# YufengJin/BundleSDF

Measured on AMD Instinct MI355X. Metric: NeRF training rays/sec + ms/iter, 64-frame pool, 2048 rays/frame, higher is better.
Workload: dtype fp16 table+MLP (MFMA) / fp32 accumulate+Adam (amp)

## Files before the change

bundlesdf_amd/csrc/field_step.hip:

```cpp
#include <algorithm>
#include <cstdlib>
#include <cstring>
#include <array>
#include <type_traits>
#include <vector>

#include "nof_device.h"
#include "ray_trace.h"
#include "mlp_lds.h"

#pragma clang fp contract(off)

#ifndef NOF_ABLATE
#define NOF_ABLATE 0
#endif
#define ABL(bits) (NOF_ABLATE && (a.ablate & (bits)))
#define ABL_HOST(d, bits) (NOF_ABLATE && ((d)->ablate & (bits)))
#define ABL_SKIPQ(q) ((q) < 2 ? (1 << (23 + (q))) : (1 << (27 + (q))))

namespace nof {

typedef _Float16 h8v __attribute__((ext_vector_type(8)));
typedef float f16v __attribute__((ext_vector_type(16)));

// ... 279 lines not shown
            const bool hit = !done && rem <= len;
            res = hit ? zin + rem : res;
            rem = done || hit ? rem : rem - len;
            done = done || hit;
            prev_out = zout;
        }
        if (!__any(!done)) return res;
    }
    for (; i < Kmax; ++i) {
        const float zin = __uint_as_float(bq[2 * i]), zout = __uint_as_float(bq[2 * i + 1]);
        if (zin == 0.f) return done ? res : ((rem <= eps && i >= 1) ? prev_out : 0.f);
        const float len = zout - zin;
        const bool hit = !done && rem <= len;
        res = hit ? zin + rem : res;
        rem = done || hit ? rem : rem - len;
        done = done || hit;
        prev_out = zout;
    }
    return done ? res : (rem <= eps ? __uint_as_float(bq[(Kmax - 1) * 2 + 1]) : 0.f);
}

__device__ __forceinline__ float bell_weight(const FieldArgs &a, float depth, float z) {
    if (depth > a.far_sc) return 0.f;
    const float u = (depth - z) / a.trunc;
    float w = sigmoidf(u * a.lambda) * sigmoidf(-u * a.lambda);
    const float dz = z - depth;
    const bool m = (dz <= a.trunc * a.ntr) && (dz >= -a.trunc);
    return m ? w : 0.f;
}

struct LevelInfo { float scale; uint32_t res, off, hs; };
__device__ __forceinline__ LevelInfo level_info(const FieldArgs &a, int lv) {
    const float4 v = a.levels[lv];
    return {v.x, __float_as_uint(v.y), __float_as_uint(v.z), __float_as_uint(v.w)};
}
__device__ __forceinline__ LevelInfo level_info_uniform(const FieldArgs &a, int lv) {
    const ConstU32 p = (ConstU32)(size_t)(a.levels + lv);
    return {__uint_as_float(p[0]), p[1], p[2], p[3]};
}

__device__ __forceinline__ __amdgpu_buffer_rsrc_t table_rsrc(const void *table) {
    return __builtin_amdgcn_make_buffer_rsrc(const_cast<void *>(table), (short)0, 0x7fffffff, 0x00020000);
}
typedef uint32_t u2v __attribute__((ext_vector_type(2)));
typedef uint32_t u4v __attribute__((ext_vector_type(4)));
__device__ __forceinline__ uint2 table_pair16(__amdgpu_buffer_rsrc_t rsrc, uint32_t row) {
    const u2v v = __builtin_amdgcn_raw_buffer_load_b64(rsrc, row * 4u, 0, 0);
    return make_uint2(v.x, v.y);
}

__device__ __forceinline__ uint32_t mul24(uint32_t a, uint32_t b) {
    uint32_t d;
    asm("v_mul_u32_u24 %0, %1, %2" : "=v"(d) : "v"(a), "v"(b));
    return d;
}
__device__ __forceinline__ uint32_t mad24(uint32_t a, uint32_t b, uint32_t c) {
    uint32_t d;
    asm("v_mad_u32_u24 %0, %1, %2, %3" : "=v"(d) : "v"(a), "v"(b), "v"(c));
    return d;
}
__device__ __forceinline__ bool level_dense_v(uint32_t rs, uint32_t hs) {
    return rs <= 1625u && mul24(mul24(rs, rs), rs) <= hs;
}
__device__ __forceinline__ uint32_t dense_base_v(uint32_t off, const uint32_t pg[3], uint32_t rs) {
    return off + pg[0] + mul24(mad24(pg[2], rs, pg[1]), rs);
}
__device__ __forceinline__ bool level_dense(uint32_t rs, uint32_t hs) { return (uint64_t)rs * rs * rs <= hs; }

__device__ __forceinline__ void corner_rows(const LevelInfo &li, const uint32_t pg[3], uint32_t rows[8]) {
    const uint32_t rs = li.res + 1;
    if (level_dense(rs, li.hs)) {
        const uint32_t base = dense_base_v(li.off, pg, rs), rs2 = rs * rs;
#pragma unroll
        for (int idx = 0; idx < 8; ++idx)
            rows[idx] = base + (idx & 1) + ((idx >> 1) & 1 ? rs : 0u) + ((idx >> 2) & 1 ? rs2 : 0u);
    } else {
#pragma unroll
        for (int idx = 0; idx < 8; ++idx) {
            uint32_t pl[3];
#pragma unroll
            for (int d = 0; d < 3; ++d) pl[d] = pg[d] + ((idx >> d) & 1);
            rows[idx] = li.off + grid_row<3>(0, false, li.hs, li.res, pl);
        }
    }
}

template <typename TT, bool PAIRED = false>
__device__ __forceinline__ void gather_level(const FieldArgs &a, const LevelInfo &li, const float x01[3], float pos[3],
                                             float e[8][2], uint32_t rows[8]) {
    const TT *tab = reinterpret_cast<const TT *>(a.table);
    uint32_t pg[3];
#pragma unroll
    for (int d = 0; d < 3; ++d) {
        pos[d] = __builtin_fmaf(x01[d], li.scale, 0.5f);
        pg[d] = (uint32_t)floorf(pos[d]);
        pos[d] -= (float)pg[d];
    }
    corner_rows(li, pg, rows);
    const uint32_t rs = li.res + 1;
    if (PAIRED && level_dense(rs, li.hs)) {
#pragma unroll
        for (int idx = 0; idx < 8; idx += 2) {
            const TT *p = tab + (size_t)rows[idx] * 2;
            if constexpr (sizeof(TT) == 4) {
                typedef float f4a __attribute__((ext_vector_type(4), aligned(8)));
                const f4a v = *reinterpret_cast<const f4a *>(p);
                e[idx][0] = v.x; e[idx][1] = v.y; e[idx + 1][0] = v.z; e[idx + 1][1] = v.w;
            } else {
                uint2 v;
                __builtin_memcpy(&v, p, 8);
                const __half2 h0 = __builtin_bit_cast(__half2, v.x), h1 = __builtin_bit_cast(__half2, v.y);
                e[idx][0] = __low2float(h0); e[idx][1] = __high2float(h0);
                e[idx + 1][0] = __low2float(h1); e[idx + 1][1] = __high2float(h1);
            }
        }
    } else {
#pragma unroll
        for (int idx = 0; idx < 8; ++idx) {
            const TT *p = tab + (size_t)rows[idx] * 2;
            if constexpr (sizeof(TT) == 4) {
                const float2 v = *reinterpret_cast<const float2 *>(p);
                e[idx][0] = v.x; e[idx][1] = v.y;
            } else {
                const __half2 v = *reinterpret_cast<const __half2 *>(p);
                e[idx][0] = __low2float(v); e[idx][1] = __high2float(v);
            }
        }
    }
}

template <typename TT>
__device__ __forceinline__ void encode_level(const FieldArgs &a, const LevelInfo &li, const float x01[3], float f[2]) {
    float pos[3], e[8][2];
    uint32_t rows[8];
    gather_level<TT, true>(a, li, x01, pos, e, rows);
    f[0] = 0.f; f[1] = 0.f;
#pragma unroll
    for (int idx = 0; idx < 8; ++idx) {
        float w = 1.f;
#pragma unroll
        for (int d = 0; d < 3; ++d) w *= ((idx >> d) & 1) ? pos[d] : 1 - pos[d];
        f[0] = __builtin_fmaf(w, e[idx][0], f[0]);
        f[1] = __builtin_fmaf(w, e[idx][1], f[1]);
    }
}

template <int CTRL> __device__ __forceinline__ int dpp_i(int v) {
    return __builtin_amdgcn_update_dpp(0, v, CTRL, 0xf, 0xf, true);
}
#define DPP_ROW_SHL(n) (0x100 + (n))
#define DPP_ROW_SHR(n) (0x110 + (n))

constexpr uint32_t SLOT_EMPTY = 0xffffffffu;

__device__ __forceinline__ uint32_t lds_cas(uint32_t *p, uint32_t key) {
    uint32_t e = SLOT_EMPTY;
    __hip_atomic_compare_exchange_strong(p, &e, key, __ATOMIC_RELAXED, __ATOMIC_RELAXED, __HIP_MEMORY_SCOPE_WORKGROUP);
    return e;
}

template <bool F16V> __device__ __forceinline__ uint32_t *slot_key(uint32_t *keys, uint32_t s) {
    return keys + (F16V ? 2 * s : s);
}
__device__ __forceinline__ void lds_add_h2(void *vals, uint32_t s, uint32_t packed) {
    __builtin_amdgcn_ds_atomic_fadd_v2f16(
        (__attribute__((address_space(3))) h2v *)(reinterpret_cast<uint32_t *>(vals) + 2 * s),
        __builtin_bit_cast(h2v, packed));
}
template <bool F16V>
__device__ __forceinline__ void lds_add(void *vals, uint32_t s, float v0, float v1) {
    if constexpr (F16V) {
        lds_add_h2(vals, s, __builtin_bit_cast(uint32_t, h2v{(_Float16)v0, (_Float16)v1}));
    } else {
        float *f = reinterpret_cast<float *>(vals) + 2 * s;
        __hip_atomic_fetch_add(f, v0, __ATOMIC_RELAXED, __HIP_MEMORY_SCOPE_WORKGROUP);
        __hip_atomic_fetch_add(f + 1, v1, __ATOMIC_RELAXED, __HIP_MEMORY_SCOPE_WORKGROUP);
    }
}

template <bool F16V>
__device__ __forceinline__ bool lds_probe(uint32_t *keys, void *vals, uint32_t mask, uint32_t key, float v0, float v1,
                                          float *g32, __half *g16) {
    uint32_t s = key;
#pragma unroll 1
    for (int p = 1; p < 16; ++p) {
        s = (s + 1) & mask;
        const uint32_t old = lds_cas(slot_key<F16V>(keys, s), key);
        if (old == SLOT_EMPTY || old == key) {
            lds_add<F16V>(vals, s, v0, v1);
            return true;
        }
    }
    if (g16) atomic_add_h2(g16 + (size_t)key * 2, v0, v1);
    else { atomic_add_f32(g32 + (size_t)key * 2, v0); atomic_add_f32(g32 + (size_t)key * 2 + 1, v1); }
    return false;
}

__device__ __forceinline__ void gather_level_t16(const FieldArgs &a, const LevelInfo &li, h2v g01, float t[8],
                                                 const uint32_t rows[8]) {
    const __half *tab = reinterpret_cast<const __half *>(a.table);
    const uint32_t rs = li.res + 1;
    if (level_dense(rs, li.hs)) {
#pragma unroll
        for (int idx = 0; idx < 8; idx += 2) {
            uint2 v;
            __builtin_memcpy(&v, tab + (size_t)rows[idx] * 2, 8);
            t[idx] = __builtin_amdgcn_fdot2(__builtin_bit_cast(h2v, v.x), g01, 0.f, false);
            t[idx + 1] = __builtin_amdgcn_fdot2(__builtin_bit_cast(h2v, v.y), g01, 0.f, false);
        }
    } else {
#pragma unroll
        for (int idx = 0; idx < 8; ++idx) {
            const uint32_t v = *reinterpret_cast<const uint32_t *>(tab + (size_t)rows[idx] * 2);
            t[idx] = __builtin_amdgcn_fdot2(__builtin_bit_cast(h2v, v), g01, 0.f, false);
        }
    }
}

template <typename TT, bool F16V>
__device__ __forceinline__ void backward_level(const FieldArgs &a, const LevelInfo &li, bool member, bool active,
                                               uint32_t part, const float x01[3], float g0, float g1, h2v g01,
                                               float gx[3], int lane, uint32_t *keys, void *vals, uint32_t mask,
                                               float *g32, __half *g16, int &n_direct) {
    float pos[3];
    uint32_t pg[3], crow[8];
#pragma unroll
    for (int d = 0; d < 3; ++d) {
        pos[d] = __builtin_fmaf(x01[d], li.scale, 0.5f);
        pg[d] = (uint32_t)pos[d];
        pos[d] = __builtin_amdgcn_fractf(pos[d]);
    }
    corner_rows(li, pg, crow);
    if (active && !a.no_dx) {
        float t[8];
        if constexpr (sizeof(TT) == 2) {
            gather_level_t16(a, li, g01, t, crow);
        } else {
            float e[8][2], pos_unused[3];
            uint32_t rows_unused[8];
            gather_level<TT, true>(a, li, x01, pos_unused, e, rows_unused);
#pragma unroll
            for (int k = 0; k < 8; ++k) t[k] = __builtin_fmaf(g1, e[k][1], g0 * e[k][0]);
        }
        float dx[4], ax[4];
#pragma unroll
        for (int j = 0; j < 4; ++j) {
            dx[j] = t[2 * j + 1] - t[2 * j];
            ax[j] = __builtin_fmaf(pos[0], dx[j], t[2 * j]);
        }
        float dy[2], by[2], ux[2];
#pragma unroll
        for (int z = 0; z < 2; ++z) {
            dy[z] = ax[2 * z + 1] - ax[2 * z];
            by[z] = __builtin_fmaf(pos[1], dy[z], ax[2 * z]);
            ux[z] = __builtin_fmaf(pos[1], dx[2 * z + 1] - dx[2 * z], dx[2 * z]);
        }
        gx[0] = __builtin_fmaf(li.scale, __builtin_fmaf(pos[2], ux[1] - ux[0], ux[0]), gx[0]);
        gx[1] = __builtin_fmaf(li.scale, __builtin_fmaf(pos[2], dy[1] - dy[0], dy[0]), gx[1]);
        gx[2] = __builtin_fmaf(li.scale, by[1] - by[0], gx[2]);
    }
    if ABL(1) return;
    const int key = member ? (int)((1u + (pg[0] | (pg[1] << 10) | (pg[2] << 20))) | (part << 31))
                           : (0x40000000 + lane + 1);
    const bool tail = member && (dpp_i<0x130>(key) != key);
    if (ABL(1 << 27)) {
        n_direct += tail ? 1 : 0;
    }
    const bool s1 = dpp_i<DPP_ROW_SHR(1)>(key) == key, s2 = dpp_i<DPP_ROW_SHR(2)>(key) == key;
    const bool s4 = dpp_i<DPP_ROW_SHR(4)>(key) == key, s8 = dpp_i<DPP_ROW_SHR(8)>(key) == key;
    const bool sb15 = __builtin_amdgcn_update_dpp(0, key, 0x142, 0xa, 0xf, false) == key;
    const bool sb31 = __builtin_amdgcn_update_dpp(0, key, 0x143, 0xc, 0xf, false) == key;
    const bool any1 = __any(s1), any2 = __any(s2);
    const bool any4 = __any(s4), any8 = __any(s8);
    const bool anyb15 = __any(sb15), anyb31 = __any(sb31);
    const float h0 = active ? g0 : 0.f, h1 = active ? g1 : 0.f;
    float wxy[4];
#pragma unroll
    for (int j = 0; j < 4; ++j) wxy[j] = ((j & 1) ? pos[0] : 1 - pos[0]) * ((j & 2) ? pos[1] : 1 - pos[1]);
    const float wz0[2] = {(1 - pos[2]) * h0, pos[2] * h0}, wz1[2] = {(1 - pos[2]) * h1, pos[2] * h1};
    float v0[8], v1[8];
#pragma unroll
    for (int idx = 0; idx < 8; ++idx) {
        v0[idx] = wxy[idx & 3] * wz0[idx >> 2];
        v1[idx] = wxy[idx & 3] * wz1[idx >> 2];
    }
    uint32_t pk[8];
    const bool pscan = F16V && !ABL(4096);
    if (pscan) {
#pragma unroll
        for (int idx = 0; idx < 8; ++idx) pk[idx] = __builtin_bit_cast(uint32_t, h2v{(_Float16)v0[idx], (_Float16)v1[idx]});
#define PFMAC_DPP(I, CTRL) "v_pk_fmac_f16_dpp %" #I ", %" #I ", %8 " CTRL "\n"
#define PSCAN_STEP(SK, CTRL)                                                                                      \
        if (any##SK) {                                                                                            \
            const uint32_t m = s##SK ? 0x3C003C00u : 0u;                                                          \
            asm("s_nop 1\n" PFMAC_DPP(0, CTRL) PFMAC_DPP(1, CTRL) PFMAC_DPP(2, CTRL) PFMAC_DPP(3, CTRL)          \
                PFMAC_DPP(4, CTRL) PFMAC_DPP(5, CTRL) PFMAC_DPP(6, CTRL) PFMAC_DPP(7, CTRL)                      \
                : "+v"(pk[0]), "+v"(pk[1]), "+v"(pk[2]), "+v"(pk[3]), "+v"(pk[4]), "+v"(pk[5]), "+v"(pk[6]),     \
                  "+v"(pk[7])                                                                                     \
                : "v"(m));                                                                                        \
        }
        PSCAN_STEP(1, "row_shr:1 row_mask:0xf bank_mask:0xf bound_ctrl:1")
        PSCAN_STEP(2, "row_shr:2 row_mask:0xf bank_mask:0xf bound_ctrl:1")
        PSCAN_STEP(4, "row_shr:4 row_mask:0xf bank_mask:0xf bound_ctrl:1")
        PSCAN_STEP(8, "row_shr:8 row_mask:0xf bank_mask:0xf bound_ctrl:1")
        PSCAN_STEP(b15, "row_bcast:15 row_mask:0xa bank_mask:0xf")
        PSCAN_STEP(b31, "row_bcast:31 row_mask:0xc bank_mask:0xf")
#undef PFMAC_DPP
#undef PSCAN_STEP
    }
#define FMAC_DPP(I, CTRL) "v_fmac_f32_dpp %" #I ", %" #I ", %16 " CTRL "\n"
#define SCAN_STEP(SK, CTRL)                                                                                       \
    if (!pscan && any##SK) {                                                                                      \
        const float m = s##SK ? 1.f : 0.f;                                                                        \
        asm("s_nop 1\n" FMAC_DPP(0, CTRL) FMAC_DPP(1, CTRL) FMAC_DPP(2, CTRL) FMAC_DPP(3, CTRL)                  \
            FMAC_DPP(4, CTRL) FMAC_DPP(5, CTRL) FMAC_DPP(6, CTRL) FMAC_DPP(7, CTRL) FMAC_DPP(8, CTRL)            \
            FMAC_DPP(9, CTRL) FMAC_DPP(10, CTRL) FMAC_DPP(11, CTRL) FMAC_DPP(12, CTRL) FMAC_DPP(13, CTRL)        \
            FMAC_DPP(14, CTRL) FMAC_DPP(15, CTRL)                                                                \
            : "+v"(v0[0]), "+v"(v0[1]), "+v"(v0[2]), "+v"(v0[3]), "+v"(v0[4]), "+v"(v0[5]), "+v"(v0[6]),         \
              "+v"(v0[7]), "+v"(v1[0]), "+v"(v1[1]), "+v"(v1[2]), "+v"(v1[3]), "+v"(v1[4]), "+v"(v1[5]),         \
              "+v"(v1[6]), "+v"(v1[7])                                                                            \
            : "v"(m));                                                                                            \
    }
    SCAN_STEP(1, "row_shr:1 row_mask:0xf bank_mask:0xf bound_ctrl:1")
    SCAN_STEP(2, "row_shr:2 row_mask:0xf bank_mask:0xf bound_ctrl:1")
    SCAN_STEP(4, "row_shr:4 row_mask:0xf bank_mask:0xf bound_ctrl:1")
    SCAN_STEP(8, "row_shr:8 row_mask:0xf bank_mask:0xf bound_ctrl:1")
    SCAN_STEP(b15, "row_bcast:15 row_mask:0xa bank_mask:0xf")
    SCAN_STEP(b31, "row_bcast:31 row_mask:0xc bank_mask:0xf")
#undef FMAC_DPP
#undef SCAN_STEP
    if (!tail) return;
    if (ABL(1 << 26)) {
        n_direct += (v0[0] + v1[7] == 12345.f || (pscan && pk[3] == 12345u)) ? 1 : 0;
        return;
    }
    if constexpr (F16V) {
        if (!pscan) {
#pragma unroll
            for (int idx = 0; idx < 8; ++idx)
                pk[idx] = __builtin_bit_cast(uint32_t, h2v{(_Float16)v0[idx], (_Float16)v1[idx]});
        }
    }
    uint32_t old[8];
#pragma unroll
    for (int idx = 0; idx < 8; ++idx) old[idx] = lds_cas(slot_key<F16V>(keys, crow[idx] & mask), crow[idx]);
    bool all_ok = true;
#pragma unroll
    for (int idx = 0; idx < 8; ++idx) {
        const bool ok = old[idx] == SLOT_EMPTY || old[idx] == crow[idx];
        all_ok = all_ok && ok;
        if constexpr (F16V) {
            lds_add_h2(vals, crow[idx] & mask, ok ? pk[idx] : 0u);
        } else {
            lds_add<F16V>(vals, crow[idx] & mask, ok ? v0[idx] : 0.f, ok ? v1[idx] : 0.f);
        }
    }
    if (__builtin_expect(__any(!all_ok), 0)) {
#pragma unroll
        for (int idx = 0; idx < 8; ++idx)
            if (!(old[idx] == SLOT_EMPTY || old[idx] == crow[idx])) {
                float u0 = v0[idx], u1 = v1[idx];
                if constexpr (F16V) {
                    const h2v q = __builtin_bit_cast(h2v, pk[idx]);
                    u0 = (float)q[0];
                    u1 = (float)q[1];
                }
                n_direct += lds_probe<F16V>(keys, vals, mask, crow[idx], u0, u1, g32, g16) ? 0 : 1;
            }
    }
}

template <bool F16V, int NJ>
__device__ __forceinline__ int flush_group(uint32_t *keys, void *vals, uint32_t s0, int lane, float *g32, __half *g16,
                                           bool no_hbm) {
    uint32_t k[NJ];
    uint32_t vb[NJ];
    float va[NJ], vc[NJ];
#pragma unroll
    for (int j = 0; j < NJ; ++j) {
        const uint32_t sl = s0 + 64 * j + lane;
        if constexpr (F16V) {
            const uint2 kv = reinterpret_cast<const uint2 *>(keys)[sl];
            k[j] = kv.x;
            vb[j] = kv.y;
        } else {
            k[j] = keys[sl];
            const float2 v = reinterpret_cast<float2 *>(vals)[sl];
            va[j] = v.x; vc[j] = v.y;
        }
    }
#pragma unroll
    for (int j = 0; j < NJ; ++j) {
        const uint32_t sl = s0 + 64 * j + lane;
        if constexpr (F16V) {
            reinterpret_cast<uint2 *>(keys)[sl] = make_uint2(0xffffffffu, 0u);
        } else {
            keys[sl] = 0xffffffffu;
            reinterpret_cast<float2 *>(vals)[sl] = make_float2(0.f, 0.f);
        }
    }
    int n = 0;
#pragma unroll
    for (int j = 0; j < NJ; ++j) {
        n += (int)__popcll(__ballot(k[j] != 0xffffffffu));
        if (k[j] != 0xffffffffu && !no_hbm) {
            if constexpr (F16V) {
                typedef _Float16 h2v __attribute__((ext_vector_type(2)));
                __builtin_amdgcn_global_atomic_fadd_v2f16((__attribute__((address_space(1))) h2v *)(g16 + (size_t)k[j] * 2),
                                                          __builtin_bit_cast(h2v, vb[j]));
            } else if (g16) {
                atomic_add_h2(g16 + (size_t)k[j] * 2, va[j], vc[j]);
            } else {
                atomic_add_f32(g32 + (size_t)k[j] * 2, va[j]);
                atomic_add_f32(g32 + (size_t)k[j] * 2 + 1, vc[j]);
            }
        }
    }
    return n;
}
template <bool F16V>
__device__ __forceinline__ int flush_table(uint32_t *keys, void *vals, uint32_t mask, int lane, float *g32,
                                           __half *g16, bool no_hbm) {
    int n = 0;
    __builtin_amdgcn_fence(__ATOMIC_SEQ_CST, "wavefront");
    if (mask + 1 >= 256) {
        for (uint32_t s0 = 0; s0 <= mask; s0 += 256) n += flush_group<F16V, 4>(keys, vals, s0, lane, g32, g16, no_hbm);
    } else if (mask + 1 == 128) {
        n = flush_group<F16V, 2>(keys, vals, 0, lane, g32, g16, no_hbm);
    } else {
        n = flush_group<F16V, 1>(keys, vals, 0, lane, g32, g16, no_hbm);
    }
    __builtin_amdgcn_fence(__ATOMIC_SEQ_CST, "wavefront");
    return n;
}

__device__ __forceinline__ int lane_level(int s, int q, int h) { return 8 * s + 4 * (q >> 1) + 2 * h + (q & 1); }

template <typename TM> struct LdsW {
    const TM *p;
    __device__ __forceinline__ typename FragT<TM>::T get(int id, int lane) const { return load_frag<TM>(p, id, lane); }
};
template <typename TM> struct LdsWt {
    typedef __attribute__((address_space(3))) const char *LdsPtr;
    LdsPtr q;
    __device__ __forceinline__ LdsWt(const TM *p, int lane, int base = 0)
        : q((LdsPtr)(reinterpret_cast<const char *>(p) + ((int64_t)lane - (int64_t)base * 64) * 8 * (int64_t)sizeof(TM))) {}
    __device__ __forceinline__ void fence() { asm volatile("" : "+v"(q)); }
    __device__ __forceinline__ typename FragT<TM>::T get(int id, int) const {
        const LdsPtr a = q + id * 64 * 8 * (int)sizeof(TM);
        typename FragT<TM>::T f;
        if constexpr (sizeof(TM) == 2) {
            f = *reinterpret_cast<__attribute__((address_space(3))) const h8v *>(a);
        } else {
            typedef float f4e __attribute__((ext_vector_type(4)));
            typedef __attribute__((address_space(3))) const f4e *L4;
            const f4e x = *reinterpret_cast<L4>(a), y = *reinterpret_cast<L4>(a + 16);
            f.v[0] = x.x; f.v[1] = x.y; f.v[2] = x.z; f.v[3] = x.w; f.v[4] = y.x; f.v[5] = y.y; f.v[6] = y.z; f.v[7] = y.w;
        }
        return f;
    }
};

template <typename TM> struct Acts {
    typename FragT<TM>::T X[2], H1[2][2], Cin[2], H3[2][2], H4[2][2];
};

template <typename TM, typename W>
__device__ __forceinline__ void mlp_sdf_net(const W &wfr, const float *wb, Acts<TM> &A, int lane, float &sdf,
                                            f16v &l2) {
    const int h = lane >> 5;
    f16v acc[2];
#pragma unroll
    for (int mt = 0; mt < 2; ++mt) {
        acc_init_bias(acc[mt], wb + 0 * 64, mt, h);
#pragma unroll
        for (int s = 0; s < 2; ++s) mma(acc[mt], wfr.get(FR_L1 + mt * 2 + s, lane), A.X[s]);
    }
#pragma unroll
    for (int t = 0; t < 2; ++t)
#pragma unroll
        for (int s = 0; s < 2; ++s) acc_to_frag<TM>(acc[t], s, true, A.H1[t][s]);
    acc_init_bias(acc[0], wb + 1 * 64, 0, h);
#pragma unroll
    for (int t = 0; t < 2; ++t)
#pragma unroll
        for (int s = 0; s < 2; ++s) mma(acc[0], wfr.get(FR_L2 + 2 * t + s, lane), A.H1[t][s]);
    float sdf_v = acc[0][0];
    if constexpr (sizeof(TM) == 2) sdf_v = (float)(_Float16)sdf_v;
    sdf = __shfl(sdf_v, lane & 31, 64);
    l2 = acc[0];
}

template <typename TM, typename W>
__device__ __forceinline__ void mlp_colour_net(const W &wfr, const float *wb, Acts<TM> &A, const f16v &l2,
                                               const typename FragT<TM>::T &shf, int lane, float logit[3], bool masks,
// ... 721 lines not shown
        }
        float s0, s1, s2, sf;
        half_sums(h == 0 ? rc[0] : rc[1], s0, s1);
        half_sums(h == 0 ? rc[2] : lf, s2, sf);
        reinterpret_cast<float4 *>(a.rrec + slot * TREC)[2] = make_float4(s0, s1, s2, sf);
        cur = nxt;
        nxt = nn;
    }
}

__global__ __launch_bounds__(256) void k_ray_final(FieldArgs a_) {
    const FieldArgs a = step_args(a_);
    const int r = blockIdx.x * blockDim.x + threadIdx.x;
    const int lane = threadIdx.x & 63, wave = threadIdx.x >> 6;
    float v[10];
#pragma unroll
    for (int k = 0; k < 10; ++k) v[k] = 0.f;
    if (r < a.R) {
        const int ntiles = a.S / 32;
        float wtot = 0.f, nvalid = 0.f, lfs = 0.f, lem = 0.f, lsdf = 0.f, lfsr = 0.f;
        float racc[3] = {0.f, 0.f, 0.f};
        int csig = 0, ccol = 0, crcol = 0, crsig = 0;
#pragma unroll 4
        for (int t = 0; t < ntiles; ++t) {
            const size_t slot = (size_t)r * ntiles + t;
            const float4 *q = reinterpret_cast<const float4 *>(a.rrec + slot * TREC);
            const float4 q0 = q[0], q1 = q[1], q2 = q[2];
            const uint8_t fl = a.tile_bwd[slot];
            wtot += q0.x; nvalid += q0.y; lfs += q0.z; lem += q0.w; lsdf += q1.x;
            const int cnt = __float_as_int(q1.y);
            csig += cnt & TC_SIG; ccol += (cnt >> 1) & 1; crcol += (cnt >> 2) & 1; crsig += (cnt >> 3) & 1;
            if (fl == 1 || fl == 3) {
                racc[0] += q2.x; racc[1] += q2.y; racc[2] += q2.z; lfsr += q2.w;
            }
        }
        const float *cx = a.rctx + (size_t)r * RCTX;
        const float tgt[3] = {cx[3], cx[4], cx[5]};
        const int frame = __float_as_int(cx[23]), rtype = __float_as_int(cx[24]);
        const bool vray = nvalid > 0.f && rtype == 0;
        const float rw = vray ? (frame == 0 ? a.ffw : 1.f) : 0.f;
        float drgb[3], lr = 0.f, rgb[3];
#pragma unroll
        for (int cc = 0; cc < 3; ++cc) {
            rgb[cc] = racc[cc] / (wtot + 1e-10f);
            const float e = rgb[cc] - tgt[cc];
            drgb[cc] = a.rgb_w * 2.f * e * rw * a.inv_3R;
            lr += e * e * rw;
        }
        v[0] = a.rgb_w * lr * a.inv_3R;
        v[1] = lfs * rw;
        v[2] = lem * rw;
        v[3] = lsdf * rw;
        v[4] = nvalid;
        v[5] = lfsr * rw;
        v[6] = (float)csig; v[7] = (float)ccol; v[8] = (float)crcol; v[9] = (float)crsig;
        if (a.dbg_rgb) {
            a.dbg_rgb[r * 3] = rgb[0]; a.dbg_rgb[r * 3 + 1] = rgb[1]; a.dbg_rgb[r * 3 + 2] = rgb[2];
        }
        float4 *ra = reinterpret_cast<float4 *>(a.ray_aux + (size_t)r * RAY_AUX);
        ra[0] = make_float4(drgb[0], drgb[1], drgb[2], wtot);
        ra[1] = make_float4(rw, 0.f, 0.f, 0.f);
        float4 *rg = reinterpret_cast<float4 *>(a.ray_grad + (size_t)r * 12);
        rg[0] = make_float4(0.f, 0.f, 0.f, 0.f);
        rg[1] = make_float4(0.f, 0.f, 0.f, 0.f);
        rg[2] = make_float4(0.f, 0.f, 0.f, 0.f);
    }
    __shared__ float s_v[4][10];
#pragma unroll
    for (int k = 0; k < 10; ++k) {
        const float t = wave_sum(v[k]);
        if (lane == 0) s_v[wave][k] = t;
    }
    __syncthreads();
    if (threadIdx.x < 10) {
        const int k = threadIdx.x;
        const float t = s_v[0][k] + s_v[1][k] + s_v[2][k] + s_v[3][k];
        constexpr int slot[10] = {0, 1, 2, 3, 4, 10, 6, 7, 8, 9};
        if (t != 0.f && (k != 5 || a.fs_rgb_w > 0.f)) atomic_add_f32(loss_row(a, (int)blockIdx.x) + slot[k], t);
    }
}

constexpr int ENCODE_GROUP_SMALL = 2;

constexpr int COMPACT_PER_BLOCK = 4096;
__global__ __launch_bounds__(256) void k_compact(const uint8_t *__restrict__ flags, int n, int *__restrict__ list,
                                                 int *__restrict__ count, int per_block, int *__restrict__ clist) {
    __shared__ int s_wave[3][4];
    __shared__ int s_base[3];
    const int lane = threadIdx.x & 63, wave = threadIdx.x >> 6;
    const int fpt = per_block >> 8;
    const int b0 = blockIdx.x * per_block + threadIdx.x * fpt;
    uint8_t fl[16];
    if (fpt == 16 && b0 + 16 <= n) {
        const uint4 v = *reinterpret_cast<const uint4 *>(flags + b0);
        const uint32_t w[4] = {v.x, v.y, v.z, v.w};
#pragma unroll
        for (int k = 0; k < 16; ++k) fl[k] = (uint8_t)(w[k >> 2] >> (8 * (k & 3)));
    } else {
#pragma unroll
        for (int k = 0; k < 16; ++k) fl[k] = (k < fpt && b0 + k < n) ? flags[b0 + k] : 0;
    }
    int mine[3] = {0, 0, 0};
#pragma unroll
    for (int k = 0; k < 16; ++k) {
        mine[0] += fl[k] == 1;
        mine[1] += fl[k] == 2;
        mine[2] += (fl[k] == 1 || fl[k] == 3);
    }
    int pm[3] = {mine[0], mine[1], mine[2]};
#pragma unroll
    for (int o = 1; o < 64; o <<= 1) {
#pragma unroll
        for (int q = 0; q < 3; ++q) {
            const int u = __shfl_up(pm[q], o, 64);
            if (lane >= o) pm[q] += u;
        }
    }
    if (lane == 63) {
#pragma unroll
        for (int q = 0; q < 3; ++q) s_wave[q][wave] = pm[q];
    }
    __syncthreads();
    if (threadIdx.x < 3) {
        const int q = threadIdx.x;
        const int tot = s_wave[q][0] + s_wave[q][1] + s_wave[q][2] + s_wave[q][3];
        int *cnt = count + (q == 0 ? 0 : (q == 1 ? 2 : 1));
        s_base[q] = (tot && (q < 2 || clist)) ? atomicAdd(cnt, tot) : 0;
    }
    __syncthreads();
    int off[3];
#pragma unroll
    for (int q = 0; q < 3; ++q) {
        off[q] = s_base[q] + pm[q] - mine[q];
        for (int w = 0; w < wave; ++w) off[q] += s_wave[q][w];
    }
#pragma unroll
    for (int k = 0; k < 16; ++k) {
        const int i = b0 + k;
        if (fl[k] == 1) list[off[0]++] = i << 5;
        if (fl[k] == 2) list[n - 1 - off[1]++] = (i << 5) | (int)0x80000000;
        if (clist && (fl[k] == 1 || fl[k] == 3)) clist[off[2]++] = i << 5;
    }
}

__device__ __forceinline__ int bwd_entry(const FieldArgs &a, int li, int n_c, int cap) {
    return a.tile_sid[li < n_c ? li : cap - 1 - (li - n_c)];
}

#include "field_mlp_bwd.h"

__device__ __forceinline__ void loss_fold(const float *__restrict__ part, float *__restrict__ loss_acc, int k);

__host__ __device__ constexpr uint32_t scatter_wave_words(uint32_t mask, int VW) {
    return (1 + VW) * (mask + 1) + 160;
}
template <typename TM, typename TT, bool F16V, int WAVES>
__global__ __launch_bounds__(256) __attribute__((amdgpu_num_sgpr(80), amdgpu_waves_per_eu(WAVES, 8))) void k_scatter(FieldArgs a_) {
    const FieldArgs a = step_args(a_);
    extern __shared__ __attribute__((aligned(16))) char smem[];
    const int lane = threadIdx.x & 63;
    const int wave = __builtin_amdgcn_readfirstlane((int)(threadIdx.x >> 6));
    if (blockIdx.x == 0 && wave == 0) loss_fold(a.loss_part, a.loss_acc, lane);
    const int bx = (a.xcd_order & 2) ? xcd_block(blockIdx.x, gridDim.x) : (int)blockIdx.x;
    const int lpw = a.scatter_lpw, ngrp = ((int)a.L + lpw - 1) / lpw;
    const int gw = __builtin_amdgcn_readfirstlane(bx * 4 + wave);
    const int r = __builtin_amdgcn_readfirstlane(gw / ngrp);
    if (r >= a.R || ABL(65536)) return;
    const int lv0 = __builtin_amdgcn_readfirstlane((gw - r * ngrp) * lpw);
    const int nlev = min(lpw, (int)a.L - lv0);
    const int ntiles = a.S / 32;
    const uint8_t *flags = a.tile_bwd + (size_t)r * ntiles;
    const uint8_t fl = lane < ntiles ? flags[lane] : (uint8_t)0;
    uint32_t gm = lane < ntiles ? a.tile_gmask[(size_t)r * ntiles + lane] : 0u;
    const bool tf = fl == 1 || fl == 2;
    if (!__any(tf) || ABL(131072)) return;
    gm = tf ? gm : 0u;
    const uint32_t mask = a.slot_mask;
    constexpr int VW = F16V ? 1 : 2;
    uint32_t *keys = reinterpret_cast<uint32_t *>(smem) + (size_t)wave * scatter_wave_words(mask, VW);
    uint32_t *vals = F16V ? keys + 1 : keys + mask + 1;
    uint16_t *slist = reinterpret_cast<uint16_t *>(keys + (1 + VW) * (mask + 1));
    if constexpr (F16V) {
        for (uint32_t s = lane; s <= mask; s += 64) reinterpret_cast<uint2 *>(keys)[s] = make_uint2(0xffffffffu, 0u);
    } else {
        for (uint32_t s = lane; s <= mask; s += 64) keys[s] = 0xffffffffu;
        for (uint32_t s = lane; s < VW * (mask + 1); s += 64) vals[s] = 0u;
    }
    if ABL(262144) return;
    float *g32 = (sizeof(TM) == 2) ? nullptr : a.grad_table;
    __half *g16 = (sizeof(TM) == 2) ? a.grad_table16 : nullptr;
    const RayCtx c = load_ray(a, r);
    int n_act = 0;
    for (int ch = 0; ch * 64 < a.S; ++ch) {
        const int s = 64 * ch + lane;
        const uint32_t m0 = (uint32_t)__builtin_amdgcn_readlane((int)gm, 2 * ch);
        const uint32_t m1 = 2 * ch + 1 < 64 ? (uint32_t)__builtin_amdgcn_readlane((int)gm, 2 * ch + 1) : 0u;
        const bool cand = s < a.S && (((lane < 32 ? m0 : m1) >> (s & 31)) & 1u);
        const uint64_t b = __ballot(cand);
        if (cand) slist[n_act + (int)__popcll(b & ((1ull << lane) - 1ull))] = (uint16_t)s;
        n_act += (int)__popcll(b);
    }
    n_act = __builtin_amdgcn_readfirstlane(n_act);
    if (n_act == 0) return;
    __builtin_amdgcn_fence(__ATOMIC_SEQ_CST, "wavefront");
    const int nch = (n_act + 63) / 64;
    float sgz[3] = {0.f, 0.f, 0.f}, sg[3] = {0.f, 0.f, 0.f};
    int n_flush = 0, n_direct = 0;
    if (!ABL(32)) {
        typedef typename std::conditional<sizeof(TM) == 2, uint32_t, float2>::type GPair;
        const size_t RS = (size_t)a.R * a.S;
        const int n_it = nlev * nch;
        auto issue = [&](int lv, int ch, float &z, GPair &g, uint32_t &prt) {
            const int j = 64 * ch + lane;
            const int sj_raw = (int)slist[j];
            const int sj = j < n_act ? sj_raw : 0;
            const size_t sid = (size_t)r * a.S + sj;
            prt = sj >= a.N_oct ? 1u : 0u;
            z = a.zbuf[sid];
            g = reinterpret_cast<const GPair *>(a.dfeat)[(size_t)lv * RS + sid];
        };
        float z_nx = 0.f;
        GPair g_nx{};
        uint32_t prt_nx = 0u;
        issue(lv0, 0, z_nx, g_nx, prt_nx);
        int lv = lv0, ch = 0, lv_n = lv0, ch_n = 0;
        for (int it = 0; it < n_it; ++it) {
            const float z = z_nx;
            const GPair gq = g_nx;
            const uint32_t part = prt_nx;
            if (++ch_n == nch) { ch_n = 0; ++lv_n; }
            issue(min(lv_n, (int)a.L - 1), ch_n, z_nx, g_nx, prt_nx);
            const bool member = 64 * ch + lane < n_act;
            float p[3], x[3], g0, g1;
            h2v g01;
            sample_point(load_ray<true>(a, r), z, p, x);
            if constexpr (sizeof(TM) == 2) {
                g01 = __builtin_bit_cast(h2v, gq);
                g0 = (float)g01[0];
                g1 = (float)g01[1];
            } else {
                g01 = h2v{(_Float16)0.f, (_Float16)0.f};
                g0 = gq.x;
                g1 = gq.y;
            }
            const bool act = member && (g0 != 0.f || g1 != 0.f);
            if (ABL(1 << 25)) {
                n_flush += __any(act) ? (int)__popcll(__ballot(act)) : 0;
                n_direct += (__any(act) && lane == 0) ? 64 : 0;
            }
            const bool skipq = ABL(ABL_SKIPQ(lv >> 2));
            if (__any(act) && !skipq) {
                const LevelInfo li = level_info_uniform(a, lv);
                const float x01[3] = {(x[0] + 1) / 2, (x[1] + 1) / 2, (x[2] + 1) / 2};
                float gx[3] = {0.f, 0.f, 0.f};
                backward_level<TT, F16V>(a, li, member, act, part, x01, g0, g1, g01, gx, lane, keys, vals, mask, g32, g16,
                                         n_direct);
#pragma unroll
                for (int i = 0; i < 3; ++i) {
                    sgz[i] = __builtin_fmaf(gx[i], z, sgz[i]);
                    sg[i] += gx[i];
                }
            }
            if (ch == nch - 1 && !ABL(1) && !ABL(1 << 22) && !skipq) {
                const int nfl = flush_table<F16V>(keys, vals, mask, lane, g32, g16, ABL(128));
                n_flush += nfl;
            }
            if (++ch == nch) { ch = 0; ++lv; }
        }
    }
    if (!a.no_dx) {
        float tz[3], t1[3];
#pragma unroll
        for (int i = 0; i < 3; ++i) {
            tz[i] = 0.5f * wave_sum(sgz[i]);
            t1[i] = 0.5f * wave_sum(sg[i]);
        }
        if (lane < 12) {
            const int i = lane >> 2, j = lane & 3;
            const float gzi = i == 0 ? tz[0] : (i == 1 ? tz[1] : tz[2]);
            const float g1i = i == 0 ? t1[0] : (i == 1 ? t1[1] : t1[2]);
            const float dj = j == 0 ? c.dir[0] : (j == 1 ? c.dir[1] : c.dir[2]);
            const float v = j < 3 ? gzi * dj : g1i;
            if (ngrp == 1) a.ray_grad[(size_t)r * 12 + lane] += v;
            else atomic_add_f32(a.ray_grad + (size_t)r * 12 + lane, v);
        }
    }
    if (!a.count_atomics || ABL(16384)) return;
    const float nf = (float)__builtin_amdgcn_readfirstlane(n_flush), nd = wave_sum((float)n_direct);
    float *cnt = a.loss_acc + 8 + 2 * (r & 63);
    if (lane == 0 && nf != 0.f) atomic_add_f32(cnt, nf);
    if (lane == 0 && nd != 0.f) atomic_add_f32(cnt + 1, nd);
}

struct QueryArgs {
    const float *pts;
    const float *gx, *gy, *gz;
    int nx, ny, nz;
    int64_t n;
    const uint8_t *occ;
    int occ_n;
    float *sdf;
};

template <typename TM, typename TT>
__global__ __launch_bounds__(256) void k_query_sdf(FieldArgs a, QueryArgs q) {
    extern __shared__ __attribute__((aligned(16))) char smem[];
    TM *s_fr = reinterpret_cast<TM *>(smem);
    float *s_b = reinterpret_cast<float *>(smem + N_FRAGS * 64 * 8 * sizeof(TM));
    {
        const uint4 *src = reinterpret_cast<const uint4 *>(a.frags);
        uint4 *dst = reinterpret_cast<uint4 *>(s_fr);
        for (int i = threadIdx.x; i < N_FRAGS * 64 * 8 * (int)sizeof(TM) / 16; i += blockDim.x) dst[i] = src[i];
        for (int i = threadIdx.x; i < 5 * 64; i += blockDim.x) s_b[i] = a.bias[i];
    }
    __syncthreads();
    const int lane = threadIdx.x & 63, n = lane & 31, h = lane >> 5;
    const int wave = __builtin_amdgcn_readfirstlane((int)(threadIdx.x >> 6));
    const int64_t ntile = (q.n + 31) / 32;
    for (int64_t t = (int64_t)blockIdx.x * 4 + wave; t < ntile; t += (int64_t)gridDim.x * 4) {
        const int64_t idx = t * 32 + n;
        const bool inb = idx < q.n;
        float x[3] = {0.f, 0.f, 0.f};
        if (inb) {
            if (q.pts) {
#pragma unroll
                for (int d = 0; d < 3; ++d) x[d] = q.pts[idx * 3 + d];
            } else {
                const int64_t k = idx % q.nz, ij = idx / q.nz;
                const int64_t j = ij % q.ny, i = ij / q.ny;
                x[0] = q.gx[i]; x[1] = q.gy[j]; x[2] = q.gz[k];
            }
        }
        bool valid = inb;
        if (inb && q.occ) {
            const float N = (float)q.occ_n;
            uint32_t c[3];
            bool inside = true;
#pragma unroll
            for (int d = 0; d < 3; ++d) {
                inside = inside && fabsf(x[d]) <= 1.f;
                const float f = floorf((x[d] + 1.f) * 0.5f * N);
                c[d] = (uint32_t)fminf(fmaxf(f, 0.f), N - 1.f);
            }
            valid = inside && q.occ[((size_t)c[2] * q.occ_n + c[1]) * q.occ_n + c[0]] != 0;
        }
        if (!__any(valid)) {
            if (inb && h == 0) q.sdf[idx] = 1.f;
            continue;
        }
#pragma unroll
        for (int d = 0; d < 3; ++d) x[d] = fminf(fmaxf(x[d], -1.f), 1.f);
        const float x01[3] = {(x[0] + 1) / 2, (x[1] + 1) / 2, (x[2] + 1) / 2};
        Acts<TM> A;
#pragma unroll
        for (int ss = 0; ss < 2; ++ss) {
#pragma unroll
            for (int qq = 0; qq < 4; ++qq) {
                const int lv = lane_level(ss, qq, h);
                float v[2] = {0.f, 0.f};
                if (inb && lv < (int)a.L) encode_level<TT>(a, level_info(a, lv), x01, v);
                frag_set<TM>(A.X[ss], 2 * qq, v[0]);
                frag_set<TM>(A.X[ss], 2 * qq + 1, v[1]);
            }
        }
        float sdf;
        f16v l2;
        mlp_sdf_net<TM>(LdsW<TM>{s_fr}, s_b, A, lane, sdf, l2);
        if (inb && h == 0) q.sdf[idx] = valid ? sdf : 1.f;
    }
}

__device__ __forceinline__ void loss_fold(const float *__restrict__ part, float *__restrict__ loss_acc, int k) {
    if (k >= LOSS_FOLD_N) return;
    constexpr int dst[LOSS_FOLD_N] = {0, 1, 2, 3, 4, 5, LOSS_ACC_COUNTERS, LOSS_ACC_COUNTERS + 1, LOSS_ACC_COUNTERS + 2,
                                      LOSS_ACC_COUNTERS + 3, LOSS_ACC_COUNTERS + 4, LOSS_ACC_COUNTERS + 5,
                                      LOSS_ACC_COUNTERS + 6};
    float s = 0.f;
    for (int c = 0; c < LOSS_COPIES; ++c) s += part[c * LOSS_SLOTS + k];
    loss_acc[dst[k]] += s;
}

__global__ __launch_bounds__(256) void k_quad_mirror(FieldArgs a) {
    __shared__ uint32_t s_off[16], s_rs[16], s_end[16];
    if (threadIdx.x < a.L) {
        const LevelInfo li = level_info(a, threadIdx.x);
        s_off[threadIdx.x] = li.off;
        s_rs[threadIdx.x] = li.res + 1;
        s_end[threadIdx.x] = level_dense(li.res + 1, li.hs) ? li.off + li.hs : 0u;
    }
    __syncthreads();
    uint32_t end = 0;
    for (int l = 0; l < (int)a.L && s_end[l]; ++l) end = s_end[l];
    const uint32_t *t = reinterpret_cast<const uint32_t *>(a.table);
    uint4 *quads = const_cast<uint4 *>(a.quads);
    int lv = 0;
    for (uint32_t i = blockIdx.x * 256u + threadIdx.x; i < end; i += gridDim.x * 256u) {
        while (lv + 1 < (int)a.L && s_off[lv + 1] <= i) ++lv;
        const uint32_t rs = s_rs[lv], hi = i + rs + 1;
        if (hi >= s_end[lv]) continue;
        quads[i] = make_uint4(t[i], t[i + 1], t[i + rs], t[hi]);
    }
}

__global__ void k_zero_i32(int *__restrict__ p, int n) {
    const int i = blockIdx.x * blockDim.x + threadIdx.x;
    if (i < n) p[i] = 0;
}

__global__ __launch_bounds__(256) void k_trace(const float *__restrict__ pool, const int32_t *__restrict__ ids, int R,
                                               const float *__restrict__ tf, const uint8_t *__restrict__ occ, int N,
                                               int Kmax, float near_sc, float far_sc, float trunc,
                                               float *__restrict__ rays_out, float *__restrict__ intervals,
                                               float *__restrict__ totals, int32_t *__restrict__ counts,
                                               const nof_step_params *__restrict__ sp,
                                               const int32_t *__restrict__ epoch_step0) {
    const int r = blockIdx.x * blockDim.x + threadIdx.x;
    if (r >= R) return;
    if (sp) trunc = sp->trunc;
    if (epoch_step0) ids += (size_t)(sp->step - *epoch_step0) * (size_t)R;
    const float *src = pool + (size_t)(ids ? ids[r] : r) * 12;
    float ray[12];
#pragma unroll
    for (int k = 0; k < 12; ++k) ray[k] = src[k];
    if (ids) {
#pragma unroll
        for (int k = 0; k < 12; ++k) rays_out[(size_t)r * 12 + k] = ray[k];
    }
    const float nrm = sqrtf((ray[0] * ray[0] + ray[1] * ray[1]) + ray[2] * ray[2]);
    const float vd[3] = {ray[0] / nrm, ray[1] / nrm, ray[2] / nrm};
    const float *T = tf + (size_t)((int)ray[8]) * 16;
    const float o[3] = {T[3], T[7], T[11]};
    float d[3];
#pragma unroll
    for (int i = 0; i < 3; ++i) d[i] = (T[i * 4] * vd[0] + T[i * 4 + 1] * vd[1]) + T[i * 4 + 2] * vd[2];
    float *dst = intervals + (size_t)r * Kmax * 2;
    const float n2 = sqrtf((vd[0] * vd[0] + vd[1] * vd[1]) + vd[2] * vd[2]);
    const float vz = fabsf(vd[2] / n2);
    const float depth = ray[6];
    const bool vdepth = (depth >= near_sc) && (depth <= far_sc);
    const float hi = depth + trunc;
// ... 455 lines not shown
```

Baseline: 29.94 million.

## Compact sparse scatter tails through LDS staging so all lanes issue atomics

In the fp16 scatter path, lanes that hold a segment tail are ballot-compacted. Each tail's 8 row keys and packed gradient values are transposed through a small per-wave LDS staging area, so every lane performs one CAS and one atomic add instead of a few lanes each doing 8 serialized ones. This aims to cut divergence and the serial LDS atomic chain when tails are sparse. It costs extra LDS words per wave, wavefront fences and staging stores. A fallback keeps the old path when there are more tails than a threshold.

```diff
diff --git a/bundlesdf_amd/csrc/field_step.hip b/bundlesdf_amd/csrc/field_step.hip
--- a/bundlesdf_amd/csrc/field_step.hip
+++ b/bundlesdf_amd/csrc/field_step.hip
@@ -455,6 +455,11 @@
 #define DPP_ROW_SHR(n) (0x110 + (n))
 
 constexpr uint32_t SLOT_EMPTY = 0xffffffffu;
+#ifndef NOF_SCATTER_TMAX
+#define NOF_SCATTER_TMAX 64
+#endif
+constexpr int SCATTER_TMAX = NOF_SCATTER_TMAX;
+constexpr uint32_t SCATTER_LIST_WORDS = 160, SCATTER_STAGE_WORDS = 64;
 
 __device__ __forceinline__ uint32_t lds_cas(uint32_t *p, uint32_t key) {
     uint32_t e = SLOT_EMPTY;
@@ -632,9 +637,12 @@
     SCAN_STEP(b31, "row_bcast:31 row_mask:0xc bank_mask:0xf")
 #undef FMAC_DPP
 #undef SCAN_STEP
-    if (!tail) return;
+    const uint64_t tmask = __ballot(tail);
+    if (ABL(1 << 28)) {
+        n_direct += (tmask != 0 && (int)__popcll(tmask) - 1 == lane) ? 1 : 0;
+    }
     if (ABL(1 << 26)) {
-        n_direct += (v0[0] + v1[7] == 12345.f || (pscan && pk[3] == 12345u)) ? 1 : 0;
+        n_direct += (tail && (v0[0] + v1[7] == 12345.f || (pscan && pk[3] == 12345u))) ? 1 : 0;
         return;
     }
     if constexpr (F16V) {
@@ -643,7 +651,47 @@
             for (int idx = 0; idx < 8; ++idx)
                 pk[idx] = __builtin_bit_cast(uint32_t, h2v{(_Float16)v0[idx], (_Float16)v1[idx]});
         }
-    }
+        const int ntail = (int)__popcll(tmask);
+        if (ntail <= SCATTER_TMAX && !ABL(1 << 20)) {
+            uint32_t *stage = keys + 2 * (mask + 1) + SCATTER_LIST_WORDS;
+            const int ti = (int)__builtin_amdgcn_mbcnt_hi((uint32_t)(tmask >> 32),
+                                                          __builtin_amdgcn_mbcnt_lo((uint32_t)tmask, 0u));
+#pragma unroll 1
+            for (int t0 = 0; t0 < ntail; t0 += 8) {
+                const bool mine = tail && ti >= t0 && ti < t0 + 8;
+                uint4 *rec = reinterpret_cast<uint4 *>(stage + 8 * ((ti - t0) & 7));
+                if (mine) {
+                    rec[0] = make_uint4(crow[0], crow[1], crow[2], crow[3]);
+                    rec[1] = make_uint4(crow[4], crow[5], crow[6], crow[7]);
+                }
+                __builtin_amdgcn_fence(__ATOMIC_SEQ_CST, "wavefront");
+                const uint32_t row = stage[lane];
+                __builtin_amdgcn_fence(__ATOMIC_SEQ_CST, "wavefront");
+                if (mine) {
+                    rec[0] = make_uint4(pk[0], pk[1], pk[2], pk[3]);
+                    rec[1] = make_uint4(pk[4], pk[5], pk[6], pk[7]);
+                }
+                __builtin_amdgcn_fence(__ATOMIC_SEQ_CST, "wavefront");
+                const uint32_t sum = stage[lane];
+                __builtin_amdgcn_fence(__ATOMIC_SEQ_CST, "wavefront");
+                const bool on = lane < 8 * (ntail - t0);
+                bool lost = false;
+                if (on) {
+                    const uint32_t o = lds_cas(slot_key<F16V>(keys, row & mask), row);
+                    lost = !(o == SLOT_EMPTY || o == row);
+                    lds_add_h2(vals, row & mask, lost ? 0u : sum);
+                }
+                if (__builtin_expect(__any(lost), 0)) {
+                    if (lost) {
+                        const h2v q = __builtin_bit_cast(h2v, sum);
+                        n_direct += lds_probe<F16V>(keys, vals, mask, row, (float)q[0], (float)q[1], g32, g16) ? 0 : 1;
+                    }
+                }
+            }
+            return;
+        }
+    }
+    if (!tail) return;
     uint32_t old[8];
 #pragma unroll
     for (int idx = 0; idx < 8; ++idx) old[idx] = lds_cas(slot_key<F16V>(keys, crow[idx] & mask), crow[idx]);
@@ -1671,7 +1719,7 @@
 __device__ __forceinline__ void loss_fold(const float *__restrict__ part, float *__restrict__ loss_acc, int k);
 
 __host__ __device__ constexpr uint32_t scatter_wave_words(uint32_t mask, int VW) {
-    return (1 + VW) * (mask + 1) + 160;
+    return (1 + VW) * (mask + 1) + SCATTER_LIST_WORDS + (VW == 1 ? SCATTER_STAGE_WORDS : 0u);
 }
 template <typename TM, typename TT, bool F16V, int WAVES>
 __global__ __launch_bounds__(256) __attribute__((amdgpu_num_sgpr(80), amdgpu_waves_per_eu(WAVES, 8))) void k_scatter(FieldArgs a_) {
@@ -1805,6 +1853,10 @@
         }
     }
     if (!a.count_atomics || ABL(16384)) return;
+    if (ABL(1 << 28)) {
+        if (n_direct != 0) atomic_add_f32(a.loss_acc + 8 + lane, (float)n_direct);
+        return;
+    }
     const float nf = (float)__builtin_amdgcn_readfirstlane(n_flush), nd = wave_sum((float)n_direct);
     float *cnt = a.loss_acc + 8 + 2 * (r & 63);
     if (lane == 0 && nf != 0.f) atomic_add_f32(cnt, nf);
```

Result: no change. 30.03 million (median of 4 runs) (+0.3%).
